# pkubioinformatics/nanoreviser

Hardware: AMD Instinct MI355X
Metric: bases revised/sec (whole node) (higher is better)
Workload: dtype f32 via scaled 2xf16 split (f32 accumulate)

## Files before the change

nanoreviser_amd/csrc/nrv_api.hip:

```cpp
#include "../../include/nanorev.h"
#include "nrv_kernels.h"
#include "nrv_tailfit.h"
#include "nrv_block.h"

#include <algorithm>
#include <cmath>
#include <cstdio>
#include <cstdlib>
#include <cstring>
#include <string>
#include <chrono>
#include <vector>

using namespace nrv;

#ifdef NRV_DEV_FAST
#define NRV_ACT1(...)
#else
#define NRV_ACT1(...) __VA_ARGS__
#endif

namespace {

thread_local std::string g_create_error = "";
// ... 813 lines not shown
  h->cap_rows = 0;
}

constexpr int kCoalesce = 4096;
static int group_windows(const nrv_handle* h) { return (h->coalesce && h->batch < kCoalesce) ? kCoalesce : h->batch; }

static int lanes_wanted(const nrv_handle* h) {
  if (h->coalesce) return 0;
  if (!h->lanes_on || h->batch > 2048 || h->batch % 32) return 0;
  const int w = 4096 / h->batch;
  return w > nrv_handle::kMaxLanes ? nrv_handle::kMaxLanes : w;
}
constexpr int kReadStageGroups = 4;
static int read_stage_groups(const nrv_handle* h) {
  static const int env = getenv("NRV_READ_STAGE") ? atoi(getenv("NRV_READ_STAGE")) : kReadStageGroups;
  return (lanes_wanted(h) > 1 || env < 1) ? 1 : (env > 8 ? 8 : env);
}
static int stage_windows(const nrv_handle* h, bool read_mode = false) {
  const int w = lanes_wanted(h);
  if (w > 1) return w * h->batch;
  return read_mode ? read_stage_groups(h) * group_windows(h) : group_windows(h);
}

static int ensure_workspace(nrv_handle* h) {
  const int T = h->T;
  const int rows = ((stage_windows(h, true) + kRowPad - 1) / kRowPad) * kRowPad;
  if (rows <= h->cap_rows) return NRV_OK;
  free_workspace(h);
  int rc;
  const size_t tiles = (size_t)(((group_windows(h) + kRowPad - 1) / kRowPad) * kRowPad) / 32;
  for (int m = 0; m < 2; ++m) {
    size_t nS = (tiles * T + 2) * 16 * 128, n1 = tiles * T * 8 * 128, n2 = tiles * T * 32 * 128,
           n3 = tiles * T * 64 * 128;
    HIPCHK(h, hipMalloc(&h->S[m], nS * 4));
    HIPCHK(h, hipMalloc(&h->X1[m], n1 * 4));
    HIPCHK(h, hipMalloc(&h->X2[m], n2 * 4));
    HIPCHK(h, hipMalloc(&h->X3[m], n3 * 4));
    HIPCHK(h, hipMalloc(&h->MO[m], tiles * T * 256 * 4));
    const size_t nm = tiles * T * 256;
    if ((rc = alloc_fill(h, h->MO[m], nm * 4)) || (rc = alloc_fill(h, h->S[m], nS * 4)) || (rc = alloc_fill(h, h->X1[m], n1 * 4)) ||
        (rc = alloc_fill(h, h->X2[m], n2 * 4)) || (rc = alloc_fill(h, h->X3[m], n3 * 4)))
      return rc;
    if (m == 0) { h->act_n[0] = nS; h->act_n[1] = n1; h->act_n[2] = n2; h->act_n[3] = n3; h->act_n[4] = nm; }
  }
  h->sig_bytes = (size_t)rows * T * kSig * 4 + 4096;
  h->feat_bytes = (size_t)rows * T * kFeat * 4 + 4096;
  for (int st = 0; st < nrv_handle::kIn; ++st) {
    HIPCHK(h, hipMalloc(&h->d_sig[st], h->sig_bytes));
    HIPCHK(h, hipMalloc(&h->d_feat[st], h->feat_bytes));
    if ((rc = poison_fill(h, h->d_sig[st], h->sig_bytes, nullptr)) || (rc = poison_fill(h, h->d_feat[st], h->feat_bytes, nullptr)))
      return rc;
  }
  for (int st = 0; st < 2; ++st) {
    const size_t ob = (size_t)rows * kOutBytes;
    HIPCHK(h, hipMalloc((void**)&h->d_out[st], ob + 64));
    HIPCHK(h, hipMemset(h->d_out[st], 0, ob + 64));
    if ((rc = poison_fill(h, h->d_out[st] + 64, ob, nullptr))) return rc;
    HIPCHK(h, hipHostMalloc((void**)&h->pin_out[st], ob + 64, hipHostMallocDefault));
    memset(h->pin_out[st], 0, ob + 64);
    h->d_p[st][0] = (float*)(h->d_out[st] + 64);
    h->d_p[st][1] = (float*)(h->d_out[st] + 64 + (size_t)rows * 24);
    h->d_a[st][0] = (int8_t*)(h->d_out[st] + 64 + (size_t)rows * 44);
    h->d_a[st][1] = (int8_t*)(h->d_out[st] + 64 + (size_t)rows * 45);
    h->d_sat_st[st] = (unsigned*)h->d_out[st];
    h->pin_sat[st] = (unsigned*)h->pin_out[st];
    h->sat_seen[st] = 0;
  }
  if (h->poison_on) HIPCHK(h, hipDeviceSynchronize());
  h->cap_rows = rows;
  return NRV_OK;
}

static void free_lanes(nrv_handle* h) {
  for (int l = 0; l < nrv_handle::kMaxLanes; ++l) {
    nrv_handle::Lane& L = h->lanes[l];
    if (L.stream) (void)hipStreamSynchronize(L.stream);
    for (int m = 0; m < 2; ++m) {
      (void)hipFree(L.S[m]); (void)hipFree(L.X1[m]); (void)hipFree(L.X2[m]); (void)hipFree(L.X3[m]); (void)hipFree(L.MO[m]);
      L.S[m] = L.X1[m] = L.X2[m] = L.X3[m] = L.MO[m] = nullptr;
    }
  }
  h->n_lanes = 0;
  h->lane_rows = 0;
}

static int ensure_lanes(nrv_handle* h) {
  const int T = h->T;
  const int rows = ((h->batch + kRowPad - 1) / kRowPad) * kRowPad;
  const int want = lanes_wanted(h);
  if (want == h->n_lanes && (want == 0 || rows <= h->lane_rows)) return NRV_OK;
  free_lanes(h);
  if (want == 0) return NRV_OK;
  const size_t tiles = rows / 32;
  const size_t nS = (tiles * T + 2) * 16 * 128, n1 = tiles * T * 8 * 128, n2 = tiles * T * 32 * 128,
               n3 = tiles * T * 64 * 128, nm = tiles * T * 256;
  if (!h->ev_fork) HIPCHK(h, hipEventCreateWithFlags(&h->ev_fork, hipEventDisableTiming));
  for (int l = 0; l < want; ++l) {
    nrv_handle::Lane& L = h->lanes[l];
    if (!L.stream) HIPCHK(h, hipStreamCreateWithFlags(&L.stream, hipStreamNonBlocking));
    if (!L.done) HIPCHK(h, hipEventCreateWithFlags(&L.done, hipEventDisableTiming));
    for (int m = 0; m < 2; ++m) {
      float** bufs[5] = {&L.S[m], &L.X1[m], &L.X2[m], &L.X3[m], &L.MO[m]};
      const size_t sz[5] = {nS, n1, n2, n3, nm};
      for (int i = 0; i < 5; ++i) {
        HIPCHK(h, hipMalloc(bufs[i], sz[i] * 4));
        const int rc = alloc_fill(h, *bufs[i], sz[i] * 4);
        if (rc) return rc;
        L.act_n[i] = sz[i];
      }
    }
  }
  HIPCHK(h, hipDeviceSynchronize());
  h->n_lanes = want;
  h->lane_rows = rows;
  return NRV_OK;
}

template <int KQ0, int KQ1, int H, int R, int WR>
static void launch_lstm_f32(nrv_handle* h, const LstmArgs& a, int tiles) {
  constexpr int NG = (H + 31) / 32;
  static_assert(NG * WR <= 4, "at most 4 waves per workgroup (one per SIMD, 512 registers each)");
#ifdef NRV_DEV_FAST
  return;
#else
  LstmArgs la = a;
  la.n_blk = (tiles + R * WR - 1) / (R * WR);
  dim3 grid(lstm_grid(la.n_blk)), blk(64 * NG * WR);
  if (h->act == 0) hipLaunchKernelGGL((lstm_layer_kernel<KQ0, KQ1, H, R, WR, false, 0>), grid, blk, 0, h->stream, la);
  NRV_ACT1(else hipLaunchKernelGGL((lstm_layer_kernel<KQ0, KQ1, H, R, WR, false, 1>), grid, blk, 0, h->stream, la);)
#endif
}


template <int KQ0, int KQ1, int H, int R, int WR>
static void launch_lstm_split(nrv_handle* h, const LstmArgs& a, const float* const ws[2], int tiles) {
  constexpr int NG = (H + 31) / 32;
#ifdef NRV_DEV_FAST
  return;
#else
  LstmSplitArgs sa;
  sa.T = a.T; sa.n_rows = a.n_rows;
  for (int m = 0; m < 2; ++m)
    sa.m[m] = LstmSplitModelParams{ws[m], a.m[m].bias, a.m[m].bn_scale, a.m[m].bn_shift, a.m[m].in0, a.m[m].in1,
                                   a.m[m].out};
  sa.n_blk = (tiles + R * WR - 1) / (R * WR);
  dim3 grid(lstm_grid(sa.n_blk)), blk(64 * NG * WR);
  if constexpr (R == 1) {
    {
      if (h->act == 0) hipLaunchKernelGGL((lstm_pair_kernel<KQ0, KQ1, H, R, WR, 0>), grid, blk, 0, h->stream, sa);
      NRV_ACT1(else hipLaunchKernelGGL((lstm_pair_kernel<KQ0, KQ1, H, R, WR, 1>), grid, blk, 0, h->stream, sa);)
      return;
    }
  }
  if constexpr (R != 1)
  {
    if (h->act == 0) hipLaunchKernelGGL((lstm_split_kernel<KQ0, KQ1, H, R, WR, 0>), grid, blk, 0, h->stream, sa);
    NRV_ACT1(else hipLaunchKernelGGL((lstm_split_kernel<KQ0, KQ1, H, R, WR, 1>), grid, blk, 0, h->stream, sa);)
  }
#endif
}

template <int KQ0, int KQ1, int H, int R, int WR, int UH, int NBG, int NA, int KBL = 0, bool RAW = false>
static void launch_lstm_h2s(nrv_handle* h, int layer, const ActView (&in0)[2], const ActView (&in1)[2],
                            float* const out[2], int T, int n, int tiles) {
  constexpr int NG = H / (16 * UH);
  LstmH2Args sa;
  sa.T = T; sa.n_rows = n;
  for (int m = 0; m < 2; ++m) {
    const DevModel& d = h->dm[m];
    sa.m[m] = LstmH2ModelParams{d.all + d.l_w2sf[layer], d.all + d.l_b2sf[layer],
                                d.all + d.l_s2[layer], d.all + d.l_h2[layer], in0[m], in1[m], out[m],
                                d.descale_f[layer]};
  }
  sa.n_blk = (tiles + R * WR - 1) / (R * WR);
  dim3 grid(lstm_grid(sa.n_blk)), blk(64 * NG * WR);
  if (h->act == 0) hipLaunchKernelGGL((lstm_h2s_kernel<KQ0, KQ1, H, R, WR, UH, 0, NBG, NA, KBL, RAW>), grid, blk, 0, h->stream, sa);
  NRV_ACT1(else hipLaunchKernelGGL((lstm_h2s_kernel<KQ0, KQ1, H, R, WR, UH, 1, NBG, NA, KBL, RAW>), grid, blk, 0, h->stream, sa);)
}

#ifndef NRV_L3_WS_NBG
#define NRV_L3_WS_NBG 4
#endif
template <int KQ0, int KQ1, int H>
static void launch_lstm_h2w(nrv_handle* h, int layer, const ActView (&in0)[2], const ActView (&in1)[2],
                            float* const out[2], int T, int n, int tiles) {
  LstmH2Args sa;
  sa.T = T; sa.n_rows = n;
  for (int m = 0; m < 2; ++m) {
    const DevModel& d = h->dm[m];
    sa.m[m] = LstmH2ModelParams{d.all + d.l_w2sf[layer], d.all + d.l_b2sf[layer], d.all + d.l_s2[layer], d.all + d.l_h2[layer],
                                in0[m], in1[m], out[m], d.descale_f[layer]};
  }
  sa.n_blk = (tiles + 1) / 2;
  dim3 grid(lstm_grid(sa.n_blk)), blk(512);
  if (h->act == 0) hipLaunchKernelGGL((lstm_h2w_kernel<KQ0, KQ1, H, 0, NRV_L3_WS_NBG>), grid, blk, 0, h->stream, sa);
  NRV_ACT1(else hipLaunchKernelGGL((lstm_h2w_kernel<KQ0, KQ1, H, 1, NRV_L3_WS_NBG>), grid, blk, 0, h->stream, sa);)
}

#if NRV_STAMP
static int g_only_stage = -1;
#define NRV_RUN_STAGE(k) (g_only_stage < 0 || g_only_stage == (k))
#else
#define NRV_RUN_STAGE(k) true
#endif

static int run_group(nrv_handle* h, const float* d_sig, const float* d_feat, int n, bool read_mode,
                     float* d_p1, float* d_p2, int8_t* d_a1, int8_t* d_a2, unsigned* sat) {
  const int T = h->T;
  const int tiles = (n + 31) / 32;
  if (h->poison_on) {
    for (int m = 0; m < 2; ++m) {
      float* const bufs[5] = {h->S[m], h->X1[m], h->X2[m], h->X3[m], h->MO[m]};
      for (int i = 0; i < 5; ++i) {
        const int rc0 = poison_fill(h, bufs[i], h->act_n[i] * 4, h->stream);
        if (rc0) return rc0;
      }
    }
  }
  hipEvent_t* ev = nullptr;
  if (h->prof && (h->prof != 3 || (h->prof_tick++ & 7) == 0)) {
    if (h->ev_used + NRV_N_KERNELS + 1 > h->ev_pool.size()) {
      for (int i = 0; i < NRV_N_KERNELS + 1; ++i) {
        hipEvent_t e;
        HIPCHK(h, hipEventCreate(&e));
        h->ev_pool.push_back(e);
      }
    }
    ev = h->ev_pool.data() + h->ev_used;
    h->ev_used += NRV_N_KERNELS + 1;
    if (h->prof == 1) HIPCHK(h, hipEventRecord(ev[0], h->stream));
  }
  auto mark = [&](int k) -> int {
    if (ev && (h->prof == 1 || k == 3 || k == 4)) HIPCHK(h, hipEventRecord(ev[k], h->stream));
    return NRV_OK;
  };
  int rc;

  bool h2_fused_l1 = false;
  {
    const int n_rows = read_mode ? n + T - 1 : n, Tc = read_mode ? 1 : T;
    const int n_tiles = read_mode ? (n + T - 1 + 31) / 32 : tiles * T;
    const int blocks = n_tiles < 128 ? n_tiles : 128;
    if (h->h2) {
      CnnRArgs a2;
      for (int m = 0; m < 2; ++m) {
        const DevModel& d = h->dm[m];
        a2.m[m] = CnnRModelParams{d.all + d.cr_w2, d.all + d.cr_ep, d.all + d.cr_d, d.all + d.cr_dbias, h->S[m]};
        a2.k[m] = d.cr_k;
      }
      a2.signal = d_sig; a2.T = Tc; a2.n_rows = n_rows; a2.n_tiles = n_tiles; a2.sat = sat;
      a2.l1_T = T; a2.l1_rows = n;
      for (int m = 0; m < 2; ++m) {
        const DevModel& d = h->dm[m];
        a2.l1[m] = Lstm1ModelParams{d.all + d.l1w16, d.all + d.l1b16, d.all + d.l1s2, d.all + d.l1h2, d_feat,
                                    read_mode ? 1 : 0, h->X1[m]};
      }
      const int wg_c = (2 * n_tiles + kCnnRWaves - 1) / kCnnRWaves, wg_l = (2 * ((n + 15) / 16) + kCnnRL1Waves - 1) / kCnnRL1Waves;
      const int wg = wg_c > wg_l ? wg_c : wg_l;
      if (!NRV_RUN_STAGE(0)) {}
      else if (h->act == 0) hipLaunchKernelGGL(cnn_r_kernel<0>, dim3(wg < 128 ? wg : 128, 2), dim3(kCnnRThreads), 0, h->stream, a2);
      NRV_ACT1(else hipLaunchKernelGGL(cnn_r_kernel<1>, dim3(wg < 128 ? wg : 128, 2), dim3(kCnnRThreads), 0, h->stream, a2);)
      h2_fused_l1 = true;
    } else {
      CnnArgs a;
      for (int m = 0; m < 2; ++m) {
        const DevModel& d = h->dm[m];
        a.m[m] = CnnModelParams{d.all + d.conv, d.all + d.dpack, d.all + d.dbias, d.all + d.dsplit, h->S[m]};
      }
      a.signal = d_sig; a.T = Tc; a.n_rows = n_rows; a.n_tiles = n_tiles;
#ifndef NRV_DEV_FAST
      if (h->split & 32) hipLaunchKernelGGL(cnn_kernel<true>, dim3(blocks, 2), dim3(kCnnThreads), 0, h->stream, a);
      else hipLaunchKernelGGL(cnn_kernel<false>, dim3(blocks, 2), dim3(kCnnThreads), 0, h->stream, a);
#endif
    }
    if ((rc = mark(1))) return rc;
  }
  auto win_view = [&](const float* p, int kq) { return ActView{p, kq, 0, T, 1}; };
  {
    LstmArgs a;
    a.T = T; a.n_rows = n;
    if (!h2_fused_l1) {
      Lstm1Args a1;
      a1.T = T; a1.n_rows = n;
      for (int m = 0; m < 2; ++m) {
        const DevModel& d = h->dm[m];
        a1.m[m] = Lstm1ModelParams{d.all + d.l1w16, d.all + d.l1b16, d.all + (h->h2 ? d.l1s2 : d.l_s[0]),
                                   d.all + (h->h2 ? d.l1h2 : d.l_h[0]), d_feat, read_mode ? 1 : 0, h->X1[m]};
      }
      dim3 grid((n + 63) / 64, 2, 2);
      if (h->h2) {
        if (h->act == 0) hipLaunchKernelGGL((lstm1_kernel<0, true>), grid, dim3(256), 0, h->stream, a1);
        NRV_ACT1(else hipLaunchKernelGGL((lstm1_kernel<1, true>), grid, dim3(256), 0, h->stream, a1);)
      } else if (h->act == 0) hipLaunchKernelGGL(lstm1_kernel<0>, grid, dim3(256), 0, h->stream, a1);
      NRV_ACT1(else hipLaunchKernelGGL(lstm1_kernel<1>, grid, dim3(256), 0, h->stream, a1);)
    }
    if ((rc = mark(2))) return rc;
    for (int m = 0; m < 2; ++m) {
      const DevModel& d = h->dm[m];
      a.m[m] = LstmModelParams{d.all + d.l_w[1], d.all + d.l_b[1], d.all + d.l_s[1], d.all + d.l_h[1],
                               win_view(h->X1[m], 8), ActView{}, nullptr, 0, h->X2[m]};
    }
    const ActView none[2] = {ActView{}, ActView{}};
    if (h->h2) {
      Lstm2TArgs ta;
      ta.T = T; ta.n_rows = n;
      for (int m = 0; m < 2; ++m) {
        const DevModel& d = h->dm[m];
        ta.m[m] = Lstm2TModelParams{d.all + d.l2t_w, d.all + d.l2t_b, h->X1[m], h->X2[m], d.descale[1]};
      }
      dim3 grid((n + 63) / 64, 2, 2);
      if (!NRV_RUN_STAGE(2)) {}
      else if (h->act == 0) hipLaunchKernelGGL(lstm2_u_kernel<0>, grid, dim3(kL2uThreads), 0, h->stream, ta);
      NRV_ACT1(else hipLaunchKernelGGL(lstm2_u_kernel<1>, grid, dim3(kL2uThreads), 0, h->stream, ta);)
    }
    else if (h->split & 2) {
      const float* ws[2] = {h->dm[0].all + h->dm[0].l_ws[1], h->dm[1].all + h->dm[1].l_ws[1]};
      launch_lstm_split<8, 0, 64, 1, 2>(h, a, ws, tiles);
    } else {
      launch_lstm_f32<8, 0, 64, 1, 2>(h, a, tiles);
    }
    if ((rc = mark(3))) return rc;
    for (int m = 0; m < 2; ++m) {
      const DevModel& d = h->dm[m];
      ActView sv = read_mode ? ActView{h->S[m], 16, 1, 1, 0} : win_view(h->S[m], 16);
      a.m[m] = LstmModelParams{d.all + d.l_w[2], d.all + d.l_b[2], d.all + d.l_s[2], d.all + d.l_h[2],
                               win_view(h->X2[m], 32), sv, nullptr, 0, h->X3[m]};
    }
    if (h->h2) {
      const ActView i0[2] = {win_view(h->X2[0], 32), win_view(h->X2[1], 32)};
      const ActView i1[2] = {read_mode ? ActView{h->S[0], 16, 1, 1, 0} : win_view(h->S[0], 16),
                             read_mode ? ActView{h->S[1], 16, 1, 1, 0} : win_view(h->S[1], 16)};
      float* const o[2] = {h->X3[0], h->X3[1]};
      if (NRV_RUN_STAGE(3)) launch_lstm_h2w<32, 16, 128>(h, 2, i0, i1, o, T, n, tiles);
    } else if (h->split & 4) {
      const float* ws[2] = {h->dm[0].all + h->dm[0].l_ws[2], h->dm[1].all + h->dm[1].l_ws[2]};
      launch_lstm_split<32, 16, 128, 2, 1>(h, a, ws, tiles);
    } else {
      launch_lstm_f32<32, 16, 128, 1, 1>(h, a, tiles);
    }
    if ((rc = mark(4))) return rc;
    for (int m = 0; m < 2; ++m) {
      const DevModel& d = h->dm[m];
      a.m[m] = LstmModelParams{d.all + d.l_w[3], d.all + d.l_b[3], d.all + d.l_s[3], d.all + d.l_h[3],
                               win_view(h->X3[m], 64), ActView{}, nullptr, 0, h->X2[m] };
    }
    if (h->h2) {
      const ActView i0[2] = {win_view(h->X3[0], 64), win_view(h->X3[1], 64)};
      float* const o[2] = {h->X2[0], h->X2[1]};
      if (NRV_RUN_STAGE(4)) launch_lstm_h2s<64, 0, 64, 2, 1, 1, 8, 2, 3, true>(h, 3, i0, none, o, T, n, tiles);
    } else if (h->split & 8) {
      const float* ws[2] = {h->dm[0].all + h->dm[0].l_ws[3], h->dm[1].all + h->dm[1].l_ws[3]};
      launch_lstm_split<64, 0, 64, 1, 2>(h, a, ws, tiles);
    } else {
      launch_lstm_f32<64, 0, 64, 1, 2>(h, a, tiles);
    }
    if ((rc = mark(5))) return rc;
  }
  {
    float* dp[2] = {d_p1 ? d_p1 : h->d_p[0][0], d_p2 ? d_p2 : h->d_p[0][1]};
    int8_t* da[2] = {d_a1 ? d_a1 : h->d_a[0][0], d_a2 ? d_a2 : h->d_a[0][1]};
    if (h->h2) {
      HeadH2Args ha;
      ha.T = T; ha.n_rows = n; ha.n_tiles = tiles;
      for (int m = 0; m < 2; ++m) {
        const DevModel& d = h->dm[m];
        ha.m[m] = HeadH2ModelParams{d.all + d.h_w2, d.all + d.h_b2, h->X2[m], d.all + d.fw8, d.all + d.fb, d.all + d.ow,
                                    d.all + d.ob, dp[m], da[m], d.hsc.c12, d.hsc.c23, d.hsc.c3o, d.C};
      }
      if (NRV_RUN_STAGE(5)) hipLaunchKernelGGL(head_h2_kernel, dim3(tiles < 128 ? tiles : 128, 2), dim3(kHeadH2Threads), 0, h->stream, ha);
      if ((rc = mark(6))) return rc;
      HIPCHK(h, hipGetLastError());
      return NRV_OK;
    }
    HeadArgs a;
    a.T = T; a.n_rows = n;
    for (int m = 0; m < 2; ++m) {
      const DevModel& d = h->dm[m];
      a.m[m] = HeadModelParams{d.all + d.d1p, d.all + d.d1b, d.all + d.d2p, d.all + d.d2b,
                               d.all + d.mop, d.all + d.mob, d.all + d.fw, d.all + d.fb,
                               d.all + d.ow, d.all + d.ob, h->X2[m], h->MO[m], dp[m], da[m], d.C};
    }
    if (h->split & 16) {
      HeadSplitArgs sa;
      sa.n_units = tiles * T;
      for (int m = 0; m < 2; ++m) {
        const DevModel& d = h->dm[m];
        sa.m[m] = HeadSplitModelParams{d.all + d.h_ws, d.all + d.h_wb, h->X2[m], h->MO[m]};
      }
      const int blocks = sa.n_units < 512 ? (sa.n_units + 3) / 4 : 128;
#ifndef NRV_DEV_FAST
      hipLaunchKernelGGL(head_mlp_split_kernel, dim3(blocks, 2), dim3(256), 0, h->stream, sa);
    } else {
      hipLaunchKernelGGL(head_mlp_kernel, dim3(tiles * T, 2), dim3(64), 0, h->stream, a);
#endif
    }
#ifndef NRV_DEV_FAST
    hipLaunchKernelGGL(head_final_kernel, dim3(tiles, 2), dim3(256), 0, h->stream, a);
#endif
    if ((rc = mark(6))) return rc;
  }
  HIPCHK(h, hipGetLastError());
  return NRV_OK;
}

static int prof_collect(nrv_handle* h) {
  if (h->ev_used == 0) return NRV_OK;
  HIPCHK(h, hipStreamSynchronize(h->stream));
  for (size_t g = 0; g + NRV_N_KERNELS + 1 <= h->ev_used; g += NRV_N_KERNELS + 1)
    for (int k = 0; k < NRV_N_KERNELS; ++k) {
      if (h->prof != 1 && k != 3) continue;
      float ms = 0.f;
      HIPCHK(h, hipEventElapsedTime(&ms, h->ev_pool[g + k], h->ev_pool[g + k + 1]));
      h->prof_ms[k] += ms;
      h->prof_n[k] += 1;
    }
  h->ev_used = 0;
  return NRV_OK;
}

static int check_handle(nrv_handle* h) {
  if (!h) return NRV_E_INVALID;
  hipError_t e = hipSetDevice(h->device);
  if (e != hipSuccess) { h->err = std::string("hipSetDevice: ") + hipGetErrorString(e); return NRV_E_HIP; }
  return NRV_OK;
}

}

extern "C" {

int nrv_create(const nrv_weights* m1, const nrv_weights* m2, int T, int device, int recurrent_act,
               nrv_handle** out) {
  if (!out) { g_create_error = "nrv_create: out is NULL"; return NRV_E_INVALID; }
  *out = nullptr;
  if (T < 1 || T > kMaxT) { g_create_error = "nrv_create: window length T out of range [1,32]"; return NRV_E_INVALID; }
  if (recurrent_act != 0 && recurrent_act != 1) { g_create_error = "nrv_create: recurrent_act must be 0 or 1"; return NRV_E_INVALID; }
  Blob b1, b2;
  if (!make_blob(m1, T, 6, &b1)) { g_create_error = "nrv_create: model1 blob size does not match the graph for this T (expect 6 classes)"; return NRV_E_WEIGHTS; }
  if (!make_blob(m2, T, 5, &b2)) { g_create_error = "nrv_create: model2 blob size does not match the graph for this T (expect 5 classes)"; return NRV_E_WEIGHTS; }
  int ndev = 0;
  hipError_t e = hipGetDeviceCount(&ndev);
  if (e != hipSuccess || ndev <= 0) {
    g_create_error = std::string("nrv_create: no HIP device (") + hipGetErrorString(e) + "); this library has no CPU fallback";
    return NRV_E_NO_DEVICE;
  }
  if (device < 0 || device >= ndev) { g_create_error = "nrv_create: device index out of range"; return NRV_E_NO_DEVICE; }
  e = hipSetDevice(device);
  if (e != hipSuccess) { g_create_error = std::string("hipSetDevice: ") + hipGetErrorString(e); return NRV_E_HIP; }
  nrv_handle* h = new (std::nothrow) nrv_handle();
  if (!h) { g_create_error = "out of host memory"; return NRV_E_NOMEM; }
  h->device = device; h->T = T; h->act = recurrent_act;
  if (const char* s = getenv("NRV_PRECISION")) {
    if (!strcmp(s, "f32")) { h->split = 0; h->h2 = 0; }
    else if (!strcmp(s, "bf16x3")) { h->split = 62; h->h2 = 0; }
    else if (!strcmp(s, "f16x2")) { h->split = 62; h->h2 = 1; }
  }
  int rc = NRV_OK;
  e = hipStreamCreateWithFlags(&h->own_stream, hipStreamDefault);
  if (e != hipSuccess) { g_create_error = std::string("hipStreamCreate: ") + hipGetErrorString(e); delete h; return NRV_E_HIP; }
  h->stream = h->own_stream;
  bool ok = hipStreamCreateWithFlags(&h->copy_stream, hipStreamNonBlocking) == hipSuccess &&
            hipStreamCreateWithFlags(&h->d2h_stream, hipStreamNonBlocking) == hipSuccess;
  for (int st = 0; st < nrv_handle::kIn && ok; ++st) ok = hipEventCreateWithFlags(&h->ev_in[st], hipEventDisableTiming) == hipSuccess;
  for (int st = 0; st < 2 && ok; ++st)
    ok = hipEventCreateWithFlags(&h->ev_done[st], hipEventDisableTiming) == hipSuccess &&
         hipEventCreateWithFlags(&h->ev_out[st], hipEventDisableTiming) == hipSuccess;
  if (const char* e2 = getenv("NRV_HOST_REGISTER")) h->host_register = atoi(e2) != 0;
  if (const char* e3 = getenv("NRV_LANES")) h->lanes_on = atoi(e3) != 0;
  if (const char* e4 = getenv("NRV_COALESCE")) h->coalesce = atoi(e4) != 0;
  if (const char* e6 = getenv("NRV_LABELS_BUDGET"); e6 && *e6) { const long long v = atoll(e6); if (v > 0) h->lab_budget = (size_t)v; }
  if (const char* e7 = getenv("NRV_FIT_MAX_ROWS"); e7 && *e7) { const long long v = atoll(e7); if (v > 0) h->fit.max_rows = v > ((long long)1 << 31) - 1 ? ((long long)1 << 31) - 1 : v; }
  if (const char* e5 = getenv("NRV_POISON"); e5 && *e5) { h->poison_on = true; h->poison = (unsigned)strtoul(e5, nullptr, 16); }
  ok = ok && hipMalloc((void**)&h->d_sat, 4 * sizeof(unsigned)) == hipSuccess &&
       hipMemset(h->d_sat, 0, 4 * sizeof(unsigned)) == hipSuccess;
  if (!ok) { g_create_error = "nrv_create: could not create the copy stream / events / counters"; nrv_destroy(h); return NRV_E_HIP; }
  if ((rc = upload_model(h, 0, b1, 6)) || (rc = upload_model(h, 1, b2, 5)) || (rc = ensure_workspace(h))) {
    g_create_error = h->err;
    nrv_destroy(h);
    return rc;
  }
  *out = h;
  return NRV_OK;
}

void nrv_destroy(nrv_handle* h) {
  if (!h) return;
  (void)hipSetDevice(h->device);
  if (h->stream) (void)hipStreamSynchronize(h->stream);
  free_workspace(h);
  free_lanes(h);
  for (int l = 0; l < nrv_handle::kMaxLanes; ++l) {
    if (h->lanes[l].done) (void)hipEventDestroy(h->lanes[l].done);
    if (h->lanes[l].stream) (void)hipStreamDestroy(h->lanes[l].stream);
  }
  if (h->ev_fork) (void)hipEventDestroy(h->ev_fork);
  for (int m = 0; m < 2; ++m) (void)hipFree(h->dm[m].all);
  for (hipEvent_t e : h->ev_pool) (void)hipEventDestroy(e);
  if (h->copy_stream) { (void)hipStreamSynchronize(h->copy_stream); (void)hipStreamDestroy(h->copy_stream); }
  if (h->d2h_stream) { (void)hipStreamSynchronize(h->d2h_stream); (void)hipStreamDestroy(h->d2h_stream); }
  if (h->edit_stream) { (void)hipStreamSynchronize(h->edit_stream); (void)hipStreamDestroy(h->edit_stream); }
  if (h->lab_stream) { (void)hipStreamSynchronize(h->lab_stream); (void)hipStreamDestroy(h->lab_stream); }
  (void)hipFree(h->d_lab);
  for (char* p : h->lab_retired) (void)hipFree(p);
  for (int m = 0; m < 2; ++m) {
    (void)hipFree(h->fit.flat[m]); (void)hipFree(h->fit.y[m]);
    (void)hipFree(h->fit.m[m].d_par); (void)hipFree(h->fit.m[m].d_state); (void)hipFree(h->fit.m[m].d_lr);
  }
  (void)hipFree(h->fit.d_partial); (void)hipFree(h->fit.d_pstat); (void)hipFree(h->fit.d_order); (void)hipFree(h->fit.d_p);
  for (int st = 0; st < nrv_handle::kIn; ++st) if (h->ev_in[st]) (void)hipEventDestroy(h->ev_in[st]);
  for (int st = 0; st < 2; ++st) {
    if (h->ev_done[st]) (void)hipEventDestroy(h->ev_done[st]);
    if (h->ev_out[st]) (void)hipEventDestroy(h->ev_out[st]);
  }
  (void)hipFree(h->d_raw); (void)hipFree(h->d_starts); (void)hipFree(h->d_reads);
  for (auto& sl : h->raw_slot) {
    (void)hipFree(sl.d_in); (void)hipFree(sl.d_out); (void)hipHostFree(sl.pin_in); (void)hipHostFree(sl.pin_out);
    (void)hipFree(sl.d_stat);
    (void)hipFree(sl.d_mrg); (void)hipHostFree(sl.pin_mrg);
    if (sl.ev_in) (void)hipEventDestroy(sl.ev_in);
    if (sl.ev_done) (void)hipEventDestroy(sl.ev_done);
    if (sl.ev_out) (void)hipEventDestroy(sl.ev_out);
  }
  (void)hipFree(h->d_sat);
  if (h->ev_raw) (void)hipEventDestroy(h->ev_raw);
  if (h->own_stream) (void)hipStreamDestroy(h->own_stream);
  delete h;
}

int nrv_set_batch(nrv_handle* h, int batch) {
  int rc = check_handle(h);
  if (rc) return rc;
  if (batch < 1 || batch > (1 << 20)) { h->err = "nrv_set_batch: batch out of range"; return NRV_E_INVALID; }
  HIPCHK(h, hipStreamSynchronize(h->stream));
  h->batch = batch;
  if ((rc = ensure_workspace(h))) return rc;
  return ensure_lanes(h);
}
int nrv_get_batch(nrv_handle* h) { return h ? h->batch : NRV_E_INVALID; }

int nrv_set_precision(nrv_handle* h, int mode) {
  int rc = check_handle(h);
  if (rc) return rc;
  if (mode != NRV_PREC_F32 && mode != NRV_PREC_BF16X3 && mode != NRV_PREC_F16X2) {
    h->err = "nrv_set_precision: unknown mode";
    return NRV_E_INVALID;
  }
  h->split = mode == NRV_PREC_F32 ? 0 : 62;
  h->h2 = mode == NRV_PREC_F16X2;
  return NRV_OK;
}
int nrv_get_precision(nrv_handle* h) {
  if (!h) return NRV_E_INVALID;
  return h->h2 ? NRV_PREC_F16X2 : (h->split ? NRV_PREC_BF16X3 : NRV_PREC_F32);
}

int nrv_set_stream(nrv_handle* h, void* s) {
  int rc = check_handle(h);
  if (rc) return rc;
  HIPCHK(h, hipStreamSynchronize(h->stream));
  h->stream = s ? (hipStream_t)s : h->own_stream;
  return NRV_OK;
}

int nrv_sync(nrv_handle* h) {
  int rc = check_handle(h);
  if (rc) return rc;
  HIPCHK(h, hipStreamSynchronize(h->stream));
  return NRV_OK;
}

}

template <class F>
static int for_groups(nrv_handle* h, int64_t n, F&& body) {
  const int64_t G = group_windows(h);
  const int64_t ng = (n + G - 1) / G;
  int nl = (h->n_lanes > 1 && ng > 1 && h->prof == 0) ? h->n_lanes : 0;
  if ((int64_t)nl > ng) nl = (int)ng;
  hipStream_t main = h->stream;
  float* keep[5][2];
  for (int m = 0; m < 2; ++m) { keep[0][m] = h->S[m]; keep[1][m] = h->X1[m]; keep[2][m] = h->X2[m]; keep[3][m] = h->X3[m]; keep[4][m] = h->MO[m]; }
  size_t keep_n[5];
  memcpy(keep_n, h->act_n, sizeof keep_n);
  auto restore = [&]() {
    for (int m = 0; m < 2; ++m) { h->S[m] = keep[0][m]; h->X1[m] = keep[1][m]; h->X2[m] = keep[2][m]; h->X3[m] = keep[3][m]; h->MO[m] = keep[4][m]; }
    memcpy(h->act_n, keep_n, sizeof keep_n);
    h->stream = main;
  };
  if (nl) {
    HIPCHK(h, hipEventRecord(h->ev_fork, main));
    for (int l = 0; l < nl; ++l) HIPCHK(h, hipStreamWaitEvent(h->lanes[l].stream, h->ev_fork, 0));
  }
  int rc = NRV_OK;
  int64_t g = 0;
  for (int64_t s = 0; s < n && !rc; s += G, ++g) {
    const int nb = (int)((n - s < G) ? (n - s) : G);
    if (nl) {
      const nrv_handle::Lane& L = h->lanes[g % nl];
      for (int m = 0; m < 2; ++m) { h->S[m] = L.S[m]; h->X1[m] = L.X1[m]; h->X2[m] = L.X2[m]; h->X3[m] = L.X3[m]; h->MO[m] = L.MO[m]; }
      memcpy(h->act_n, L.act_n, sizeof L.act_n);
      h->stream = L.stream;
    }
    rc = body(s, nb);
  }
  restore();
  if (nl) {
    for (int l = 0; l < nl; ++l) {
      hipError_t e = hipEventRecord(h->lanes[l].done, h->lanes[l].stream);
      if (e == hipSuccess) e = hipStreamWaitEvent(main, h->lanes[l].done, 0);
      if (e != hipSuccess && !rc) { h->err = std::string("lane join: ") + hipGetErrorString(e); rc = NRV_E_HIP; }
    }
  }
  return rc;
}

template <class Begin>
// ... 2298 lines not shown
```

nanoreviser_amd/csrc/nrv_lstm2_u.h:

```cpp
#pragma once
#include "nrv_lstm_f16x2s.h"

namespace nrv {

constexpr int kL2uThreads = 512;

struct Lstm2TModelParams {
  const void* wfrag;
  const float* bias;
  const float* in;
  float* out;
  float descale;
};
struct Lstm2TArgs {
  Lstm2TModelParams m[2];
  int T;
  int n_rows;
};

typedef float f32x2 __attribute__((ext_vector_type(2)));
typedef _Float16 f16x2 __attribute__((ext_vector_type(2)));

constexpr int kL2tWFrags = 3 * 16 * 2;

__device__ __forceinline__ void lstm2_t_stage(const Lstm2TModelParams& P, const int dir, float* wl, float* bl,
                                              const int tid, const int nthreads) {
  const __amdgpu_buffer_rsrc_t wrs = make_rsrc((const char*)P.wfrag + (size_t)dir * kL2tWFrags * 1024, kL2tWFrags * 1024);
  for (int base = 0; base < kL2tWFrags * 64; base += 8 * nthreads) {
    f32x4 v[8];
#pragma unroll
    for (int j = 0; j < 8; ++j) v[j] = buf_load16(wrs, (unsigned)(base + j * nthreads + tid) * 16, 0);
#pragma unroll
    for (int j = 0; j < 8; ++j)
      if (base + j * nthreads + tid < kL2tWFrags * 64) ((f32x4*)wl)[base + j * nthreads + tid] = v[j];
  }
  const f32x4* bsrc = (const f32x4*)(P.bias + (size_t)dir * 16 * 256);
  for (int i = tid; i < 16 * 64; i += nthreads) ((f32x4*)bl)[i] = bsrc[i];
}


template <int ACT>
__device__ __forceinline__ void lstm2_u_unit(const Lstm2TModelParams& P, const int T, const int dir, const int rb,
                                             const int lane, const int hf, const float* wl, const float* bl, f32x4* hx) {
  constexpr int NR = 4, LEAD = 3;
  const int n = lane & 15, q = lane >> 4;
  const int tile = rb >> 1, trow = 16 * (rb & 1) + n;
  const float dsc = P.descale, dsc02 = 0.2f * dsc, dsc2 = 2.885390081777927f * dsc;
  const __amdgpu_buffer_rsrc_t xrs = make_rsrc(P.in + (size_t)tile * T * 8 * 128, (unsigned)T * 8 * 512);
  const unsigned xv = (unsigned)((4 * (q >> 1) + (q & 1)) * 512 + trow * 16);
  auto t_of = [&](int s) __attribute__((always_inline)) { const int sc = s < T ? s : T - 1; return dir ? (T - 1 - sc) : sc; };
  struct XFrag { f32x4 hi, lo; };
  auto load_x = [&](int s) __attribute__((always_inline)) {
    XFrag x;
    const unsigned so = (unsigned)t_of(s) * 8 * 512;
    x.lo = __builtin_bit_cast(f32x4, __builtin_amdgcn_raw_buffer_load_b128(xrs, xv + 1024, so, 0));
    x.hi = __builtin_bit_cast(f32x4, __builtin_amdgcn_raw_buffer_load_b128(xrs, xv, so, 0));
    return x;
  };
  float* const obase = P.out + ((size_t)tile * T * 32 + (dir * 4) * 4 + (q >> 1)) * 128 + trow * 4 + (q & 1) * 2 + (size_t)hf * 2 * 4 * 128;
  const float* const wlh = wl + hf * 2 * 2 * 256 + lane * 4;
  const float* const blh = bl + hf * 2 * 256 + lane * 4;

  struct WPair { f32x4 hi, lo; };
  WPair wr[NR];
  auto frag_of = [&](int ci) __attribute__((always_inline)) {
    if (ci < 16) { const int u = ci >> 3, g = (ci >> 1) & 3, kb = 1 + (ci & 1); return ((kb * 16) + g * 4 + u) * 2; }
    const int u = (ci - 16) >> 2, g = (ci - 16) & 3;
    return (g * 4 + u) * 2;
  };
  auto load_w = [&](int ci) __attribute__((always_inline)) {
    const int f = frag_of(ci);
    wr[ci % NR].lo = *(const f32x4*)(wlh + (f + 1) * 256);
    wr[ci % NR].hi = *(const f32x4*)(wlh + f * 256);
  };

  f32x4 Z[8];
  float c[8];
  f16x8 hB[2][2];
  f16x8 hN[2];
#pragma unroll
  for (int i = 0; i < 8; ++i) c[i] = 0.f;

  constexpr int GST = 13;
  struct GateSt { float zi, zf, zg, zo, cp, p, t; };
  GateSt gsr;
  float hv[4];
  auto gate_stage = [&](int u, int r, int st, int t_out) __attribute__((always_inline)) {
    const int e = 4 * u + r;
    GateSt& gs = gsr;
    if (st == 0) { gs.zi = Z[0 + u][r]; gs.zf = Z[2 + u][r]; gs.cp = c[e]; }
    else if (st == 1) { gs.zg = Z[4 + u][r]; gs.zo = Z[6 + u][r]; }
    else if (st == 2) {
      if constexpr (ACT == 0) {
        gs.zi = __builtin_fminf(__builtin_fmaxf(__builtin_fmaf(gs.zi, dsc02, 0.5f), 0.0f), 1.0f);
        gs.zf = __builtin_fminf(__builtin_fmaxf(__builtin_fmaf(gs.zf, dsc02, 0.5f), 0.0f), 1.0f);
      } else {
        gs.zi = sigmoid_exact(gs.zi * dsc);
        gs.zf = sigmoid_exact(gs.zf * dsc);
      }
    } else if (st == 3) {
      if constexpr (ACT == 0) gs.zo = __builtin_fminf(__builtin_fmaxf(__builtin_fmaf(gs.zo, dsc02, 0.5f), 0.0f), 1.0f);
      else gs.zo = sigmoid_exact(gs.zo * dsc);
      gs.zg = gs.zg * dsc2;
    } else if (st == 4) gs.zg = __builtin_amdgcn_exp2f(gs.zg);
    else if (st == 5) gs.t = __builtin_amdgcn_rcpf(gs.zg + 1.0f);
    else if (st == 6) gs.p = gs.zi * __builtin_fmaf(gs.t, -2.0f, 1.0f);
    else if (st == 7) {
      const float cn = __builtin_fmaf(gs.zf, gs.cp, gs.p);
      c[e] = cn;
      gs.zg = cn * 2.885390081777927f;
    } else if (st == 8) gs.zg = __builtin_amdgcn_exp2f(gs.zg);
    else if (st == 9) gs.t = __builtin_amdgcn_rcpf(gs.zg + 1.0f);
    else if (st == 10) hv[r] = gs.zo * __builtin_fmaf(gs.t, -2.0f * kHScale, kHScale);
    else if (st == 11) {
      if (r & 1) {
        const f16x2 hp = __builtin_convertvector(f32x2{hv[r - 1], hv[r]}, f16x2);
        hN[0][4 * u + r - 1] = hp[0];
        hN[0][4 * u + r] = hp[1];
      }
    } else {
      if (r & 1) {
        const int j = 4 * u + r;
        const f16x2 lp = __builtin_convertvector(
            f32x2{hv[r - 1] - (float)hN[0][j - 1], hv[r] - (float)hN[0][j]}, f16x2);
        hN[1][j - 1] = lp[0];
        hN[1][j] = lp[1];
      }
      if (r == 3) {
        typedef _Float16 f16x4v __attribute__((ext_vector_type(4)));
        float* d = obase + ((size_t)t_out * 32 + u * 4) * 128;
        const f16x8 a = hN[0], b = hN[1];
        const int o = 4 * u;
        *(f16x4v*)d = f16x4v{a[o], a[o + 1], a[o + 2], a[o + 3]};
        *(f16x4v*)(d + 2 * 128) = f16x4v{b[o], b[o + 1], b[o + 2], b[o + 3]};
      }
    }
  };
  auto gate_piece = [&](int u, int pc, int t_out) __attribute__((always_inline)) { gate_stage(u, pc / GST, pc % GST, t_out); };
  auto gates_plain = [&](int u, int t_out) __attribute__((always_inline)) {
#pragma unroll
    for (int pc = 0; pc < 4 * GST; ++pc) {
      gate_piece(u, pc, t_out);
      if ((pc & 3) == 3) __builtin_amdgcn_sched_barrier(0);
    }
  };
  constexpr int NGP = 4 * GST;
  constexpr int PA[3] = {0, 0, 1}, PB[3] = {0, 1, 0};

  auto rec_phase = [&](int t_out) __attribute__((always_inline)) {
#pragma unroll
    for (int ci = 0; ci < 16; ++ci) {
      const int u = ci >> 3, g = (ci >> 1) & 3, kb = ci & 1;
      load_w(ci + LEAD);
      __builtin_amdgcn_sched_barrier(0);
#pragma unroll
      for (int pr = 0; pr < 3; ++pr) {
        const f16x8 a = __builtin_bit_cast(f16x8, PA[pr] ? wr[ci % NR].lo : wr[ci % NR].hi);
        Z[g * 2 + u] = mfma16_f16(a, hB[kb][PB[pr]], Z[g * 2 + u]);
        if (u > 0) {
          const int tk = (ci & 7) * 3 + pr;
#pragma unroll
          for (int pc = (tk * NGP) / 24; pc < ((tk + 1) * NGP) / 24; ++pc) gate_piece(0, pc, t_out);
        }
        __builtin_amdgcn_sched_barrier(0);
      }
    }
  };
  auto in_phase = [&](auto gates1_tag, const XFrag& x, int t_out) __attribute__((always_inline)) {
    constexpr bool GATES1 = decltype(gates1_tag)::value;
    const f16x8 xb[2] = {__builtin_bit_cast(f16x8, x.hi), __builtin_bit_cast(f16x8, x.lo)};
#pragma unroll
    for (int g = 0; g < 4; ++g) Z[g * 2] = *(const f32x4*)(blh + (g * 4) * 256);
#pragma unroll
    for (int k = 0; k < 8; ++k) {
      const int ci = 16 + k, u = k >> 2, g = k & 3;
      load_w(ci + LEAD < 24 ? ci + LEAD : ci + LEAD - 24);
      if (k == 4) {
#pragma unroll
        for (int gg = 0; gg < 4; ++gg) Z[gg * 2 + 1] = *(const f32x4*)(blh + (gg * 4 + 1) * 256);
      }
      __builtin_amdgcn_sched_barrier(0);
#pragma unroll
      for (int pr = 0; pr < 3; ++pr) {
        const f16x8 a = __builtin_bit_cast(f16x8, PA[pr] ? wr[ci % NR].lo : wr[ci % NR].hi);
        Z[g * 2 + u] = mfma16_f16(a, xb[PB[pr]], Z[g * 2 + u]);
        if constexpr (GATES1) {
          const int tk = k * 3 + pr;
          if (tk < 12) {
#pragma unroll
            for (int pc = (tk * NGP) / 12; pc < ((tk + 1) * NGP) / 12; ++pc) gate_piece(1, pc, t_out);
          }
        }
        __builtin_amdgcn_sched_barrier(0);
      }
    }
  };
  auto exchange = [&](int p) __attribute__((always_inline)) {
    f32x4* const img = hx + p * 4 * 64 + lane;
    img[(hf * 2 + 0) * 64] = __builtin_bit_cast(f32x4, hN[0]);
    img[(hf * 2 + 1) * 64] = __builtin_bit_cast(f32x4, hN[1]);
    __syncthreads();
#pragma unroll
    for (int kb = 0; kb < 2; ++kb)
#pragma unroll
      for (int tm = 0; tm < 2; ++tm) hB[kb][tm] = __builtin_bit_cast(f16x8, img[(kb * 2 + tm) * 64]);
  };

  XFrag xn = load_x(1);
  {
    const XFrag x0 = load_x(0);
#pragma unroll
    for (int i = 0; i < LEAD; ++i) load_w(16 + i);
    in_phase(std::false_type{}, x0, 0);
#pragma unroll
    for (int i = 0; i < LEAD; ++i) load_w(16 + i);
  }
  {
    const int t0 = t_of(0);
    gates_plain(0, t0);
    if (T > 1) {
      const XFrag x = xn;
      xn = load_x(2);
      in_phase(std::true_type{}, x, t0);
      exchange(0);
    } else {
      gates_plain(1, t0);
    }
  }
#pragma unroll 1
  for (int s = 1; s < T; ++s) {
    const int t = t_of(s);
    rec_phase(t);
    if (s + 1 < T) {
      const XFrag x = xn;
      xn = load_x(s + 2);
      in_phase(std::true_type{}, x, t);
      exchange(s & 1);
    } else {
      gates_plain(1, t);
    }
  }
}

template <int ACT>
__global__ void __launch_bounds__(kL2uThreads) lstm2_u_kernel(const Lstm2TArgs args) {
  __shared__ __attribute__((aligned(16))) float wl[kL2tWFrags * 256];
  __shared__ __attribute__((aligned(16))) float bl[16 * 256];
  __shared__ __attribute__((aligned(16))) f32x4 hx[4 * 2 * 4 * 64];
  const Lstm2TModelParams& P = args.m[blockIdx.z];
  const int lane = threadIdx.x & 63;
  const int wave = __builtin_amdgcn_readfirstlane(threadIdx.x >> 6);
  const int chain = wave & 3, hf = wave >> 2;
  lstm2_t_stage(P, blockIdx.y, wl, bl, threadIdx.x, kL2uThreads);
  __syncthreads();
  lstm2_u_unit<ACT>(P, args.T, blockIdx.y, blockIdx.x * 4 + chain, lane, hf, wl, bl, hx + chain * 2 * 4 * 64);
}

}
```

Before: 12.32 million.

## Restructure LSTM2 recurrence to register-resident weights with two interleaved row tiles

Replaces the 512-thread LSTM2 kernel that staged all weights and biases in LDS with a 256-thread kernel. Each wave keeps its slice of the weight fragments and bias in registers and processes two row sub-tiles alternately, so one tile's MFMA work overlaps the other's hidden-state exchange. Gate math is interleaved with MFMAs through sched_group_barrier, and waves_per_eu is fixed at 2. The grid doubles to keep the same total work. This removes per-step LDS weight reads and the large LDS footprint, at the cost of high register pressure and a per-half-step block barrier.

After: 12.49 million, median of 6. 1.01x the previous value.

```diff
diff --git a/nanoreviser_amd/csrc/nrv_api.hip b/nanoreviser_amd/csrc/nrv_api.hip
--- a/nanoreviser_amd/csrc/nrv_api.hip
+++ b/nanoreviser_amd/csrc/nrv_api.hip
@@ -1139,16 +1139,16 @@
     }
     const ActView none[2] = {ActView{}, ActView{}};
     if (h->h2) {
-      Lstm2TArgs ta;
+      Lstm2RArgs ta;
       ta.T = T; ta.n_rows = n;
       for (int m = 0; m < 2; ++m) {
         const DevModel& d = h->dm[m];
-        ta.m[m] = Lstm2TModelParams{d.all + d.l2t_w, d.all + d.l2t_b, h->X1[m], h->X2[m], d.descale[1]};
+        ta.m[m] = Lstm2RModelParams{d.all + d.l2t_w, d.all + d.l2t_b, h->X1[m], h->X2[m], d.descale[1]};
       }
-      dim3 grid((n + 63) / 64, 2, 2);
+      dim3 grid(2 * ((n + 63) / 64), 2, 2);
       if (!NRV_RUN_STAGE(2)) {}
-      else if (h->act == 0) hipLaunchKernelGGL(lstm2_u_kernel<0>, grid, dim3(kL2uThreads), 0, h->stream, ta);
-      NRV_ACT1(else hipLaunchKernelGGL(lstm2_u_kernel<1>, grid, dim3(kL2uThreads), 0, h->stream, ta);)
+      else if (h->act == 0) hipLaunchKernelGGL(lstm2_r_kernel<0>, grid, dim3(kL2rThreads), 0, h->stream, ta);
+      NRV_ACT1(else hipLaunchKernelGGL(lstm2_r_kernel<1>, grid, dim3(kL2rThreads), 0, h->stream, ta);)
     }
     else if (h->split & 2) {
       const float* ws[2] = {h->dm[0].all + h->dm[0].l_ws[1], h->dm[1].all + h->dm[1].l_ws[1]};
diff --git a/nanoreviser_amd/csrc/nrv_lstm2_u.h b/nanoreviser_amd/csrc/nrv_lstm2_u.h
--- a/nanoreviser_amd/csrc/nrv_lstm2_u.h
+++ b/nanoreviser_amd/csrc/nrv_lstm2_u.h
@@ -3,80 +3,66 @@
 
 namespace nrv {
 
-constexpr int kL2uThreads = 512;
-
-struct Lstm2TModelParams {
+constexpr int kL2rThreads = 256;
+
+struct Lstm2RModelParams {
   const void* wfrag;
   const float* bias;
   const float* in;
   float* out;
   float descale;
 };
-struct Lstm2TArgs {
-  Lstm2TModelParams m[2];
+struct Lstm2RArgs {
+  Lstm2RModelParams m[2];
   int T;
   int n_rows;
 };
 
 typedef float f32x2 __attribute__((ext_vector_type(2)));
 typedef _Float16 f16x2 __attribute__((ext_vector_type(2)));
-
-constexpr int kL2tWFrags = 3 * 16 * 2;
-
-__device__ __forceinline__ void lstm2_t_stage(const Lstm2TModelParams& P, const int dir, float* wl, float* bl,
-                                              const int tid, const int nthreads) {
-  const __amdgpu_buffer_rsrc_t wrs = make_rsrc((const char*)P.wfrag + (size_t)dir * kL2tWFrags * 1024, kL2tWFrags * 1024);
-  for (int base = 0; base < kL2tWFrags * 64; base += 8 * nthreads) {
-    f32x4 v[8];
-#pragma unroll
-    for (int j = 0; j < 8; ++j) v[j] = buf_load16(wrs, (unsigned)(base + j * nthreads + tid) * 16, 0);
-#pragma unroll
-    for (int j = 0; j < 8; ++j)
-      if (base + j * nthreads + tid < kL2tWFrags * 64) ((f32x4*)wl)[base + j * nthreads + tid] = v[j];
-  }
-  const f32x4* bsrc = (const f32x4*)(P.bias + (size_t)dir * 16 * 256);
-  for (int i = tid; i < 16 * 64; i += nthreads) ((f32x4*)bl)[i] = bsrc[i];
-}
-
+typedef _Float16 f16x4 __attribute__((ext_vector_type(4)));
+
+constexpr int kL2rWFrags = 3 * 16 * 2;
 
 template <int ACT>
-__device__ __forceinline__ void lstm2_u_unit(const Lstm2TModelParams& P, const int T, const int dir, const int rb,
-                                             const int lane, const int hf, const float* wl, const float* bl, f32x4* hx) {
-  constexpr int NR = 4, LEAD = 3;
+__device__ __forceinline__ void lstm2_r_chain(const Lstm2RModelParams& P, const int T, const int dir, const int tile,
+                                              const int lane, const int w, char* hx) {
   const int n = lane & 15, q = lane >> 4;
-  const int tile = rb >> 1, trow = 16 * (rb & 1) + n;
   const float dsc = P.descale, dsc02 = 0.2f * dsc, dsc2 = 2.885390081777927f * dsc;
+
+  f32x4 Wr[3][4][2];
+  f32x4 bias[4];
+  const __amdgpu_buffer_rsrc_t wrs = make_rsrc((const char*)P.wfrag + (size_t)dir * kL2rWFrags * 1024, kL2rWFrags * 1024);
+  auto load_wblock = [&](int kb) __attribute__((always_inline)) {
+#pragma unroll
+    for (int g = 0; g < 4; ++g)
+#pragma unroll
+      for (int tm = 0; tm < 2; ++tm)
+        Wr[kb][g][tm] = buf_load16(wrs, (unsigned)lane * 16, (unsigned)(((kb * 16 + g * 4 + w) * 2 + tm) * 1024));
+  };
+  load_wblock(0);
+  {
+    const __amdgpu_buffer_rsrc_t brs = make_rsrc(P.bias + (size_t)dir * 16 * 256, 16 * 1024);
+#pragma unroll
+    for (int g = 0; g < 4; ++g) bias[g] = buf_load16(brs, (unsigned)lane * 16, (unsigned)((g * 4 + w) * 1024));
+  }
+
   const __amdgpu_buffer_rsrc_t xrs = make_rsrc(P.in + (size_t)tile * T * 8 * 128, (unsigned)T * 8 * 512);
-  const unsigned xv = (unsigned)((4 * (q >> 1) + (q & 1)) * 512 + trow * 16);
+  const unsigned xv = (unsigned)((4 * (q >> 1) + (q & 1)) * 512 + n * 16);
   auto t_of = [&](int s) __attribute__((always_inline)) { const int sc = s < T ? s : T - 1; return dir ? (T - 1 - sc) : sc; };
   struct XFrag { f32x4 hi, lo; };
-  auto load_x = [&](int s) __attribute__((always_inline)) {
+  auto load_x = [&](int rt, int s) __attribute__((always_inline)) {
     XFrag x;
     const unsigned so = (unsigned)t_of(s) * 8 * 512;
-    x.lo = __builtin_bit_cast(f32x4, __builtin_amdgcn_raw_buffer_load_b128(xrs, xv + 1024, so, 0));
-    x.hi = __builtin_bit_cast(f32x4, __builtin_amdgcn_raw_buffer_load_b128(xrs, xv, so, 0));
+    x.lo = __builtin_bit_cast(f32x4, __builtin_amdgcn_raw_buffer_load_b128(xrs, xv + rt * 256 + 1024, so, 0));
+    x.hi = __builtin_bit_cast(f32x4, __builtin_amdgcn_raw_buffer_load_b128(xrs, xv + rt * 256, so, 0));
     return x;
   };
-  float* const obase = P.out + ((size_t)tile * T * 32 + (dir * 4) * 4 + (q >> 1)) * 128 + trow * 4 + (q & 1) * 2 + (size_t)hf * 2 * 4 * 128;
-  const float* const wlh = wl + hf * 2 * 2 * 256 + lane * 4;
-  const float* const blh = bl + hf * 2 * 256 + lane * 4;
-
-  struct WPair { f32x4 hi, lo; };
-  WPair wr[NR];
-  auto frag_of = [&](int ci) __attribute__((always_inline)) {
-    if (ci < 16) { const int u = ci >> 3, g = (ci >> 1) & 3, kb = 1 + (ci & 1); return ((kb * 16) + g * 4 + u) * 2; }
-    const int u = (ci - 16) >> 2, g = (ci - 16) & 3;
-    return (g * 4 + u) * 2;
-  };
-  auto load_w = [&](int ci) __attribute__((always_inline)) {
-    const int f = frag_of(ci);
-    wr[ci % NR].lo = *(const f32x4*)(wlh + (f + 1) * 256);
-    wr[ci % NR].hi = *(const f32x4*)(wlh + f * 256);
-  };
+  float* const obase = P.out + ((size_t)tile * T * 32 + (dir * 4 + w) * 4 + (q >> 1)) * 128 + n * 4 + (q & 1) * 2;
 
   f32x4 Z[8];
   float c[8];
-  f16x8 hB[2][2];
+  f16x8 hB[2][2][2];
   f16x8 hN[2];
 #pragma unroll
   for (int i = 0; i < 8; ++i) c[i] = 0.f;
@@ -127,12 +113,11 @@
         hN[1][j] = lp[1];
       }
       if (r == 3) {
-        typedef _Float16 f16x4v __attribute__((ext_vector_type(4)));
-        float* d = obase + ((size_t)t_out * 32 + u * 4) * 128;
+        float* d = obase + (size_t)t_out * 32 * 128 + u * 16 * 4;
         const f16x8 a = hN[0], b = hN[1];
         const int o = 4 * u;
-        *(f16x4v*)d = f16x4v{a[o], a[o + 1], a[o + 2], a[o + 3]};
-        *(f16x4v*)(d + 2 * 128) = f16x4v{b[o], b[o + 1], b[o + 2], b[o + 3]};
+        *(f16x4*)d = f16x4{a[o], a[o + 1], a[o + 2], a[o + 3]};
+        *(f16x4*)(d + 2 * 128) = f16x4{b[o], b[o + 1], b[o + 2], b[o + 3]};
       }
     }
   };
@@ -147,113 +132,111 @@
   constexpr int NGP = 4 * GST;
   constexpr int PA[3] = {0, 0, 1}, PB[3] = {0, 1, 0};
 
-  auto rec_phase = [&](int t_out) __attribute__((always_inline)) {
-#pragma unroll
-    for (int ci = 0; ci < 16; ++ci) {
-      const int u = ci >> 3, g = (ci >> 1) & 3, kb = ci & 1;
-      load_w(ci + LEAD);
-      __builtin_amdgcn_sched_barrier(0);
-#pragma unroll
-      for (int pr = 0; pr < 3; ++pr) {
-        const f16x8 a = __builtin_bit_cast(f16x8, PA[pr] ? wr[ci % NR].lo : wr[ci % NR].hi);
-        Z[g * 2 + u] = mfma16_f16(a, hB[kb][PB[pr]], Z[g * 2 + u]);
-        if (u > 0) {
-          const int tk = (ci & 7) * 3 + pr;
-#pragma unroll
-          for (int pc = (tk * NGP) / 24; pc < ((tk + 1) * NGP) / 24; ++pc) gate_piece(0, pc, t_out);
-        }
-        __builtin_amdgcn_sched_barrier(0);
-      }
-    }
-  };
-  auto in_phase = [&](auto gates1_tag, const XFrag& x, int t_out) __attribute__((always_inline)) {
-    constexpr bool GATES1 = decltype(gates1_tag)::value;
+  auto half = [&](auto rec_tag, auto gates_tag, int ug, int rp, const XFrag& x, int t_out) __attribute__((always_inline)) {
+    constexpr bool REC = decltype(rec_tag)::value, GATES = decltype(gates_tag)::value;
+    constexpr int NM = 12 + (REC ? 24 : 0);
+    auto pieces = [&](int tk) __attribute__((always_inline)) {
+      if constexpr (GATES) {
+#pragma unroll
+        for (int pc = (tk * NGP) / NM; pc < ((tk + 1) * NGP) / NM; ++pc) gate_piece(ug, pc, t_out);
+      }
+    };
     const f16x8 xb[2] = {__builtin_bit_cast(f16x8, x.hi), __builtin_bit_cast(f16x8, x.lo)};
 #pragma unroll
-    for (int g = 0; g < 4; ++g) Z[g * 2] = *(const f32x4*)(blh + (g * 4) * 256);
-#pragma unroll
-    for (int k = 0; k < 8; ++k) {
-      const int ci = 16 + k, u = k >> 2, g = k & 3;
-      load_w(ci + LEAD < 24 ? ci + LEAD : ci + LEAD - 24);
-      if (k == 4) {
-#pragma unroll
-        for (int gg = 0; gg < 4; ++gg) Z[gg * 2 + 1] = *(const f32x4*)(blh + (gg * 4 + 1) * 256);
-      }
-      __builtin_amdgcn_sched_barrier(0);
-#pragma unroll
-      for (int pr = 0; pr < 3; ++pr) {
-        const f16x8 a = __builtin_bit_cast(f16x8, PA[pr] ? wr[ci % NR].lo : wr[ci % NR].hi);
-        Z[g * 2 + u] = mfma16_f16(a, xb[PB[pr]], Z[g * 2 + u]);
-        if constexpr (GATES1) {
-          const int tk = k * 3 + pr;
-          if (tk < 12) {
-#pragma unroll
-            for (int pc = (tk * NGP) / 12; pc < ((tk + 1) * NGP) / 12; ++pc) gate_piece(1, pc, t_out);
+    for (int pr = 0; pr < 3; ++pr)
+#pragma unroll
+      for (int g = 0; g < 4; ++g) {
+        const f16x8 a = __builtin_bit_cast(f16x8, Wr[0][g][PA[pr]]);
+        Z[g * 2 + rp] = mfma16_f16(a, xb[PB[pr]], pr == 0 ? bias[g] : Z[g * 2 + rp]);
+        pieces(pr * 4 + g);
+      }
+    if constexpr (REC) {
+#pragma unroll
+      for (int kb = 0; kb < 2; ++kb)
+#pragma unroll
+        for (int pr = 0; pr < 3; ++pr)
+#pragma unroll
+          for (int g = 0; g < 4; ++g) {
+            const f16x8 a = __builtin_bit_cast(f16x8, Wr[1 + kb][g][PA[pr]]);
+            Z[g * 2 + rp] = mfma16_f16(a, hB[rp][kb][PB[pr]], Z[g * 2 + rp]);
+            pieces(12 + (kb * 3 + pr) * 4 + g);
           }
-        }
-        __builtin_amdgcn_sched_barrier(0);
-      }
-    }
-  };
-  auto exchange = [&](int p) __attribute__((always_inline)) {
-    f32x4* const img = hx + p * 4 * 64 + lane;
-    img[(hf * 2 + 0) * 64] = __builtin_bit_cast(f32x4, hN[0]);
-    img[(hf * 2 + 1) * 64] = __builtin_bit_cast(f32x4, hN[1]);
+    }
+#pragma unroll
+    for (int i = 0; i < NM; i += 3) {
+      __builtin_amdgcn_sched_group_barrier(0x008, 1, 0);
+      if constexpr (GATES) __builtin_amdgcn_sched_group_barrier(0x402, 3, 0);
+      __builtin_amdgcn_sched_group_barrier(0x008, 1, 0);
+      if constexpr (GATES) __builtin_amdgcn_sched_group_barrier(0x402, 2, 0);
+      __builtin_amdgcn_sched_group_barrier(0x008, 1, 0);
+      if constexpr (GATES) __builtin_amdgcn_sched_group_barrier(0x402, 2, 0);
+    }
+    __builtin_amdgcn_sched_barrier(0);
+  };
+  auto exchange = [&](int rt) __attribute__((always_inline)) {
+    char* const img = hx + rt * 4 * 1024 + lane * 16;
+#pragma unroll
+    for (int tm = 0; tm < 2; ++tm) {
+      const f16x8 v = hN[tm];
+      *(f16x4*)(img + ((w >> 1) * 2 + tm) * 1024 + (w & 1) * 8) = f16x4{v[4 * rt], v[4 * rt + 1], v[4 * rt + 2], v[4 * rt + 3]};
+    }
     __syncthreads();
 #pragma unroll
     for (int kb = 0; kb < 2; ++kb)
 #pragma unroll
-      for (int tm = 0; tm < 2; ++tm) hB[kb][tm] = __builtin_bit_cast(f16x8, img[(kb * 2 + tm) * 64]);
-  };
-
-  XFrag xn = load_x(1);
+      for (int tm = 0; tm < 2; ++tm)
+        hB[rt][kb][tm] = __builtin_bit_cast(f16x8, *(const f32x4*)(img + (kb * 2 + tm) * 1024));
+    __builtin_amdgcn_sched_barrier(0);
+  };
+  using No = std::false_type;
+  using Yes = std::true_type;
+
+  XFrag xn[2];
   {
-    const XFrag x0 = load_x(0);
-#pragma unroll
-    for (int i = 0; i < LEAD; ++i) load_w(16 + i);
-    in_phase(std::false_type{}, x0, 0);
-#pragma unroll
-    for (int i = 0; i < LEAD; ++i) load_w(16 + i);
+    const XFrag x0[2] = {load_x(0, 0), load_x(1, 0)};
+    xn[0] = load_x(0, 1);
+    xn[1] = load_x(1, 1);
+    load_wblock(1);
+    load_wblock(2);
+    half(No{}, No{}, 0, 0, x0[0], 0);
+    half(No{}, No{}, 0, 1, x0[1], 0);
+  }
+  const int t0 = t_of(0);
+  if (T == 1) {
+    gates_plain(0, t0);
+    gates_plain(1, t0);
+    return;
+  }
+  gates_plain(0, t0);
+  exchange(0);
+  half(Yes{}, Yes{}, 1, 0, xn[0], t0);
+  xn[0] = load_x(0, 2);
+  exchange(1);
+#pragma unroll 1
+  for (int s = 1; s + 1 < T; ++s) {
+    const int t = t_of(s);
+    half(Yes{}, Yes{}, 0, 1, xn[1], t);
+    xn[1] = load_x(1, s + 1);
+    exchange(0);
+    half(Yes{}, Yes{}, 1, 0, xn[0], t);
+    xn[0] = load_x(0, s + 2);
+    exchange(1);
   }
   {
-    const int t0 = t_of(0);
-    gates_plain(0, t0);
-    if (T > 1) {
-      const XFrag x = xn;
-      xn = load_x(2);
-      in_phase(std::true_type{}, x, t0);
-      exchange(0);
-    } else {
-      gates_plain(1, t0);
-    }
-  }
-#pragma unroll 1
-  for (int s = 1; s < T; ++s) {
-    const int t = t_of(s);
-    rec_phase(t);
-    if (s + 1 < T) {
-      const XFrag x = xn;
-      xn = load_x(s + 2);
-      in_phase(std::true_type{}, x, t);
-      exchange(s & 1);
-    } else {
-      gates_plain(1, t);
-    }
+    const int t = t_of(T - 1);
+    half(Yes{}, Yes{}, 0, 1, xn[1], t);
+    gates_plain(1, t);
   }
 }
 
 template <int ACT>
-__global__ void __launch_bounds__(kL2uThreads) lstm2_u_kernel(const Lstm2TArgs args) {
-  __shared__ __attribute__((aligned(16))) float wl[kL2tWFrags * 256];
-  __shared__ __attribute__((aligned(16))) float bl[16 * 256];
-  __shared__ __attribute__((aligned(16))) f32x4 hx[4 * 2 * 4 * 64];
-  const Lstm2TModelParams& P = args.m[blockIdx.z];
+__global__ void __launch_bounds__(kL2rThreads) __attribute__((amdgpu_waves_per_eu(2, 2)))
+lstm2_r_kernel(const Lstm2RArgs args) {
+  __shared__ __attribute__((aligned(16))) char hx[2 * 4 * 1024];
+  const Lstm2RModelParams& P = args.m[blockIdx.z];
   const int lane = threadIdx.x & 63;
   const int wave = __builtin_amdgcn_readfirstlane(threadIdx.x >> 6);
-  const int chain = wave & 3, hf = wave >> 2;
-  lstm2_t_stage(P, blockIdx.y, wl, bl, threadIdx.x, kL2uThreads);
-  __syncthreads();
-  lstm2_u_unit<ACT>(P, args.T, blockIdx.y, blockIdx.x * 4 + chain, lane, hf, wl, bl, hx + chain * 2 * 4 * 64);
+  lstm2_r_chain<ACT>(P, args.T, blockIdx.y, blockIdx.x, lane, wave, hx);
 }
 
 }
```
